# CAMMA-public/SelfPose3d

Measured on AMD Instinct MI355X. Metric: multi-view samples/sec (5-view Panoptic, 80x80x20 voxel), higher is better.
Workload: dtype f32

## Files before the change

### include/sp3d.h

```cpp
#ifndef SP3D_H
#define SP3D_H

#include <stdint.h>

#ifdef __cplusplus
extern "C" {
#endif

#define SP3D_ABI_VERSION 3
#define SP3D_MAX_VIEWS 16
#define SP3D_MAX_TOPK 32

#define SP3D_CAM_STRIDE 64
#define SP3D_CAM_R 0
#define SP3D_CAM_T 9
#define SP3D_CAM_F 12
#define SP3D_CAM_C 14
#define SP3D_CAM_K 16
#define SP3D_CAM_P 19
#define SP3D_CAM_A 21
#define SP3D_CAM_W0 27
#define SP3D_CAM_H0 28
#define SP3D_CAM_FLIP 29
#define SP3D_CAM_RXY 32
// ... 145 lines not shown
int sp3d_wino_input(const float *x, float *V, int B, int X, int Y, int Z, int C, void *stream);
int sp3d_wino_output(const float *M, float *y, const float *shift, const float *residual, int mode, int B, int X, int Y,
                     int Z, int O, void *stream);
int sp3d_wino_fused(const float *x, const float *U, float *y, const float *shift, const float *residual, int mode, int B,
                    int X, int Y, int Z, int C, int O, void *stream);

int sp3d_wino_fused_split(const float *x, const void *U3, float *y, const float *shift, const float *residual, int mode, int B,
                          int X, int Y, int Z, int C, int O, void *stream);

int sp3d_wino_fused_split64(const float *x, const void *U3, float *y, const float *shift, const float *residual, int mode,
                            int B, int X, int Y, int Z, int C, int O, void *stream);

int sp3d_conv3_split(const float *x, const void *W3, float *y, const float *shift, const float *residual, int mode, int B,
                     int X, int Y, int Z, int C, int O, void *stream);

int sp3d_upsample2x_scatter(const float *G, float *out, const float *shift, const float *skip, int64_t batch, int X, int Y,
                            int Z, int O, void *stream);

int sp3d_upsample2x_scatter_head(const float *G, float *head, const float *shift, const float *skip, const float *wout,
                                 const float *bout, int64_t batch, int X, int Y, int Z, int O, int J, void *stream);

#include "sp3d_upconv.h"

#define SP3D_GBN_F32 0
#define SP3D_GBN_F64 1
#define SP3D_GBN_REPLICAS 16
#define SP3D_GBN_PLAIN 0
#define SP3D_GBN_RELU 1
#define SP3D_GBN_ADD_RELU 2
int64_t sp3d_gbn_workspace_bytes(int G, int C);
// ... 14 lines not shown
```

### selfpose3d_amd/_lib.py

```python
from __future__ import annotations

import ctypes as C
import os
from typing import Optional, Sequence

import torch

_HERE = os.path.dirname(os.path.abspath(__file__))
_DEFAULT_LIB_PATH = os.path.join(_HERE, "libsp3d.so")
NOPK_LIB_PATH = os.path.join(_HERE, "libsp3d_nopk.so")
LIB_PATH = os.environ.get("SP3D_LIB_PATH") or _DEFAULT_LIB_PATH

LAYOUT_PLANAR = 0
LAYOUT_NHWC = 1
OUT_CHANNELS_LAST = 0x100
HM_BF16 = 0x200
OUT_BF16 = 0x400
HM_ONE_CHANNEL = 0x800
SCATTER_AUTO, SCATTER_PER_TAP, SCATTER_MERGE = 0, 2, 3
MAX_VIEWS = 16
MAX_TOPK = 32
ABI_VERSION = 3

_CTYPES = {"p": C.c_void_p, "i": C.c_int, "l": C.c_int64, "f": C.c_float, "d": C.c_double, "s": C.c_char_p}
# ... 53 lines not shown
}
TUNING_SIGNATURES = {
    "sp3d_unproject_fwd_variant": "i: p i ppppp iiiiiiii p iii p",
    "sp3d_unproject_fwd_plan": "i: iii p iiiiiiiii pppp",
    "sp3d_debug_set_timeline": "i: p",
    "sp3d_debug_stamp": "i: pp",
}
ONE_TRAIN_SIGNATURES = {
    "sp3d_unproject_one_fwd_train": "i: p ii ppppppp iiiiiiii p ii p",
    "sp3d_unproject_one_bwd": "i: ppppp l pp iiiiiiii p ii p",
    "sp3d_unproject_one_bwd_det": "i: ppppp l ppp iiiiiiii p ii p",
}
UPCONV_SIGNATURES = {
    "sp3d_upconv2x_fused": "i: ppppppp l iiiiii p",
}
EXPORTS = list(SIGNATURES)

_lib = None


class Sp3dError(RuntimeError):
    pass


def shared_gpu() -> bool:
    v = os.environ.get("SP3D_SHARED_GPU")
    if v is not None:
        return v.lower() in ("1", "true", "yes", "on")
    if any(os.environ.get(k) not in (None, "") for k in ("HIP_VISIBLE_DEVICES", "CUDA_VISIBLE_DEVICES", "ROCR_VISIBLE_DEVICES",
                                                          "GPU_DEVICE_ORDINAL")):
# ... 9 lines not shown
        pass
    return False


def load():
    global _lib, LIB_PATH
    if _lib is not None:
        return _lib
    if shared_gpu() and LIB_PATH == _DEFAULT_LIB_PATH:
        LIB_PATH = NOPK_LIB_PATH
    if not os.path.exists(LIB_PATH):
        raise Sp3dError(
            f"{LIB_PATH} not found - the HIP extension is not built. Run `python -m selfpose3d_amd.build` "
            "(hipcc, gfx950). There is no CPU fallback for the unprojection path.")
    lib = C.CDLL(LIB_PATH)
    for table, required in ((SIGNATURES, True), (ONE_TRAIN_SIGNATURES, True), (UPCONV_SIGNATURES, True),
                            (TUNING_SIGNATURES, False)):
        for name, sig in table.items():
            if required or hasattr(lib, name):
                ret, args = sig.split(":")
                fn = getattr(lib, name)
                fn.restype = _CTYPES[ret]
                fn.argtypes = [_CTYPES[a] for a in args.replace(" ", "")]
    if lib.sp3d_abi_version() != ABI_VERSION:
        raise Sp3dError(f"libsp3d.so ABI {lib.sp3d_abi_version()} != binding ABI {ABI_VERSION}; rebuild")
    _lib = lib
    return lib


def check(rc: int, what: str):
    if rc != 0:
# ... 603 lines not shown


def wino_weights_split(U: torch.Tensor, chunk: int = 8) -> torch.Tensor:
    P, Cc, O = (int(v) for v in U.shape)
    U = U.float()
    hi = U.bfloat16()
    r = U - hi.float()
    mid = r.bfloat16()
    lo = (r - mid.float()).bfloat16()
    pieces = torch.stack([mid, hi, lo], 0).reshape(3, P, Cc // chunk, chunk // 4, 4, O)
    return pieces.permute(1, 2, 3, 5, 0, 4).contiguous()


def conv_weights_split(w: torch.Tensor) -> torch.Tensor:
    O, Cc = int(w.shape[0]), int(w.shape[1])
    pc = wino_weights_split(w.float().permute(4, 3, 2, 1, 0).reshape(27, Cc, O).contiguous(), 8)
    mid, hi, lo = pc[..., 0, :], pc[..., 1, :], pc[..., 2, :]
    return torch.stack([hi, lo, hi, hi, mid, mid], -2).contiguous()


def conv3_split_(x: torch.Tensor, W3: torch.Tensor, shift: torch.Tensor, mode: int,
                 residual: Optional[torch.Tensor] = None) -> torch.Tensor:
    lib = load()
    _require_cuda(x, "x")
    B, Cc, X, Y, Z = (int(v) for v in x.shape)
    _require_cl3d_f32(x, "conv3_split_")
    O = int(W3.shape[3])
    dev = x.device
    y = _empty_cl3d(B, O, X, Y, Z, dev)
    if residual is not None:
        residual = _as_cl3d(residual)
    check(lib.sp3d_conv3_split(x.data_ptr(), W3.data_ptr(), y.data_ptr(), shift.data_ptr(), _opt(residual), int(mode),
                               B, X, Y, Z, Cc, O, _stream(dev)), "sp3d_conv3_split")
    return y


def wino_conv3d_(x: torch.Tensor, U: torch.Tensor, shift: torch.Tensor, mode: int,
                 residual: Optional[torch.Tensor] = None) -> torch.Tensor:
    lib = load()
    _require_cuda(x, "x")
    B, Cc, X, Y, Z = (int(v) for v in x.shape)
    _require_cl3d_f32(x, "wino_conv3d_")
    O = int(U.shape[2])
    T = B * ((X + 1) // 2) * ((Y + 1) // 2) * ((Z + 1) // 2)
    V = torch.empty((64, T, Cc), dtype=torch.float32, device=x.device)
    check(lib.sp3d_wino_input(x.data_ptr(), V.data_ptr(), B, X, Y, Z, Cc, _stream(x.device)), "sp3d_wino_input")
    M = torch.bmm(V, U)
    y = _empty_cl3d(B, O, X, Y, Z, x.device)
    if residual is not None:
        residual = _as_cl3d(residual)
    check(lib.sp3d_wino_output(M.data_ptr(), y.data_ptr(), shift.data_ptr(), _opt(residual), int(mode), B, X, Y, Z, O,
                               _stream(x.device)), "sp3d_wino_output")
    return y


def wino_fused_conv3d_(x: torch.Tensor, U: torch.Tensor, shift: torch.Tensor, mode: int,
                       residual: Optional[torch.Tensor] = None, U3: Optional[torch.Tensor] = None) -> torch.Tensor:
    lib = load()
    _require_cuda(x, "x")
    B, Cc, X, Y, Z = (int(v) for v in x.shape)
    _require_cl3d_f32(x, "wino_fused_conv3d_")
    O = int(U.shape[2])
    y = _empty_cl3d(B, O, X, Y, Z, x.device)
    if residual is not None:
        residual = _as_cl3d(residual)
    if U3 is None:
        name, weights = "sp3d_wino_fused", U
    else:
        name, weights = ("sp3d_wino_fused_split64" if O == 64 else "sp3d_wino_fused_split"), U3
    check(getattr(lib, name)(x.data_ptr(), weights.data_ptr(), y.data_ptr(), shift.data_ptr(), _opt(residual), int(mode),
                             B, X, Y, Z, Cc, O, _stream(x.device)), name)
    return y


def upconv_weights_split(w_gemm: torch.Tensor) -> torch.Tensor:
    Cc, O = int(w_gemm.shape[0]), int(w_gemm.shape[1]) // 8
    U = w_gemm.float().reshape(Cc, 8 * O // 32, 32).permute(1, 0, 2).contiguous()
    pc = wino_weights_split(U, 8)
# ... 92 lines not shown
```

### selfpose3d_amd/build.py

```python
from __future__ import annotations

import os
import subprocess
import sys

HERE = os.path.dirname(os.path.abspath(__file__))
CSRC = os.path.join(HERE, "csrc")
SOURCES = ["sp3d_unproject.hip", "sp3d_proposal.hip", "sp3d_epilogue.hip", "sp3d_upconv.hip", "sp3d_synth.hip", "sp3d_fftconv.hip", "sp3d_winograd.hip", "sp3d_fft.hip", "sp3d_gbn.hip"]
HEADERS = [os.path.join("..", "pk_src1.py"), "sp3d_device.h", "sp3d_proj_pk.h", "sp3d_split.h", "sp3d_tuning.h", "sp3d_twiddles.h", os.path.join("..", "..", "include", "sp3d.h"),
           os.path.join("..", "..", "include", "sp3d_one_train.h"), os.path.join("..", "..", "include", "sp3d_upconv.h")]
LIB = os.path.join(HERE, "libsp3d.so")
HIPCC = os.environ.get("HIPCC", "/opt/rocm/bin/hipcc")
FLAGS = ["--offload-arch=gfx950", "-O3", "-std=c++17", "-ffp-contract=off", "-munsafe-fp-atomics", "-fPIC", "-shared",
         "-Wall", "-Wno-unused-function"]
LINK = ["-L/opt/rocm/lib", "-lhipfft"]


def needs_build() -> bool:
    if not os.path.exists(LIB):
        return True
    t = os.path.getmtime(LIB)
    deps = [os.path.join(CSRC, s) for s in SOURCES + HEADERS] + [os.path.abspath(__file__)]
    return any(os.path.getmtime(d) > t for d in deps if os.path.exists(d))


# ... 102 lines not shown
```

### selfpose3d_amd/csrc/sp3d_winograd.hip

```cpp
#include <hip/hip_runtime.h>
#include <stdint.h>

#include "../../include/sp3d.h"
#include "sp3d_split.h"

namespace sp3d {

__device__ __forceinline__ void bt4(float &d0, float &d1, float &d2, float &d3)
{
    const float t0 = d0 - d2, t1 = d1 + d2, t2 = d2 - d1, t3 = d1 - d3;
    d0 = t0; d1 = t1; d2 = t2; d3 = t3;
}

__global__ __launch_bounds__(256) void wino_input_kernel(const float *__restrict__ x, float *__restrict__ V, int B, int X,
                                                        int Y, int Z, int C, int TX, int TY, int TZ)
{
    const int64_t T = (int64_t)B * TX * TY * TZ;
    const int64_t gid = (int64_t)blockIdx.x * 256 + threadIdx.x;
    if (gid >= T * C) return;
    const int c = (int)(gid % C);
    int64_t t = gid / C;
    const int tz = (int)(t % TZ); int64_t r = t / TZ;
    const int ty = (int)(r % TY); r /= TY;
    const int tx = (int)(r % TX);
// ... 526 lines not shown
                float val = acc[a][v] + sh;
                if (MODE == 2) val += rv[v];
                if (MODE >= 1) val = fmaxf(val, 0.0f);
                if (MODE == 3) val += rv[v];
                y[idx] = val;
            }
        }
    }
}

typedef float f32x4 __attribute__((ext_vector_type(4)));
constexpr int W16_RX = 10, W16_RY = 10, W16_RZ = 4, W16_VS = 16;
constexpr int W16_ROW = W16_RX * W16_VS + 4;
constexpr int W16_LDS = W16_RY * W16_RZ * W16_ROW;

__device__ __forceinline__ f32x4 mfma16_bf16(u32x4 a, u32x4 b, f32x4 c)
{
    return __builtin_amdgcn_mfma_f32_16x16x32_bf16(__builtin_bit_cast(bf16x8, a), __builtin_bit_cast(bf16x8, b), c, 0, 0, 0);
}

template <int C, int MODE, int NBW, int KS>
__global__ __launch_bounds__(64 * (4 / NBW) * KS) __attribute__((amdgpu_waves_per_eu(NBW <= 2 ? 2 : 1))) void wino_fused16_kernel(const float *__restrict__ x,
                                                                          const unsigned *__restrict__ U3,
                                                                          float *__restrict__ y, const float *__restrict__ shift,
                                                                          const float *__restrict__ res, int B, int X, int Y,
                                                                          int Z, int NBX, int NBY, int NBZ)
{
    constexpr int O = 64, NCH = C / 16, NOW = 4 / NBW, NTG = 64 * NOW;
    static_assert(NCH % KS == 0, "chunks must divide evenly over the channel groups");
    __shared__ __attribute__((aligned(16))) float lds[KS * W16_LDS];
    const int tid = threadIdx.x, lane = tid & 63, wave = tid >> 6;
    const int kg = wave / NOW, ow = wave % NOW, tg = tid - kg * NTG;
    float *region = lds + kg * W16_LDS;
    const int tl = lane & 15, q = lane >> 4;
    int bid = blockIdx.x;
    const int bz = bid % NBZ; bid /= NBZ;
    const int by = bid % NBY; bid /= NBY;
    const int bx = bid % NBX;
    const int b = bid / NBX;
    const int ttx = tl & 3, tty = tl >> 2;
    const int ox0 = bx * 8, oy0 = by * 8, oz0 = bz * 2;
// ... 146 lines not shown
                for (int bc = 0; bc < 4; ++bc) {
#if defined(SP3D_NO_PK) || defined(SP3D_W16_SCALAR_ACC)
                    for (int e = 0; e < 4; ++e) {
                        acc[bc][n][e] = fmaf(M0[n][e], cyz[bc], acc[bc][n][e]);
                        acc[4 + bc][n][e] = fmaf(M1[n][e], cyz[bc], acc[4 + bc][n][e]);
                    }
#else
                    const f32x4 cv = {cyz[bc], cyz[bc], cyz[bc], cyz[bc]};
                    acc[bc][n] = __builtin_elementwise_fma(M0[n], cv, acc[bc][n]);
                    acc[4 + bc][n] = __builtin_elementwise_fma(M1[n], cv, acc[4 + bc][n]);
#endif
                }
        }
    }

    if (KS > 1) {
        __syncthreads();
        f32x4 *red = reinterpret_cast<f32x4 *>(lds);
        if (kg > 0) {
#pragma unroll
            for (int a = 0; a < 8; ++a)
#pragma unroll
                for (int n = 0; n < NBW; ++n) red[(((kg - 1) * NOW + ow) * 8 * NBW + a * NBW + n) * 64 + lane] = acc[a][n];
        }
        __syncthreads();
        if (kg > 0) return;
#pragma unroll
        for (int g2 = 1; g2 < KS; ++g2)
#pragma unroll
            for (int a = 0; a < 8; ++a)
// ... 12 lines not shown
            for (int v = 0; v < 4; ++v) off[v] = ((2 * v * Y + 2 * q) * Z) * O;
            float rv[8][4];
            if (MODE >= 2) {
#pragma unroll
                for (int a = 0; a < 8; ++a)
#pragma unroll
                    for (int v = 0; v < 4; ++v)
                        rv[a][v] = res[obase + off[v] + (((a >> 2) * Y + ((a >> 1) & 1)) * Z + (a & 1)) * O];
            }
#pragma unroll
            for (int a = 0; a < 8; ++a)
#pragma unroll
                for (int v = 0; v < 4; ++v) {
                    float val = acc[a][n][v] + sh;
                    if (MODE == 2) val += rv[a][v];
                    if (MODE >= 1) val = fmaxf(val, 0.0f);
                    if (MODE == 3) val += rv[a][v];
                    y[obase + off[v] + (((a >> 2) * Y + ((a >> 1) & 1)) * Z + (a & 1)) * O] = val;
                }
        }
        return;
    }
#pragma unroll
    for (int n = 0; n < NBW; ++n) {
        const int o = (ow * NBW + n) * 16 + tl;
        const float sh = shift[o];
        float rv[8][4];
        if (MODE >= 2) {
#pragma unroll
            for (int a = 0; a < 8; ++a)
#pragma unroll
// ... 4 lines not shown
                    const int zo = min(oz0 + (a & 1), Z - 1);
                    rv[a][v] = res[((((int64_t)b * X + xo) * Y + yo) * Z + zo) * O + o];
                }
        }
#pragma unroll
        for (int a = 0; a < 8; ++a) {
#pragma unroll
            for (int v = 0; v < 4; ++v) {
                const int tile = 4 * q + v;
                const int rx = tile & 3, ry = tile >> 2;
                const int xo = ox0 + 2 * rx + (a >> 2), yo = oy0 + 2 * ry + ((a >> 1) & 1), zo = oz0 + (a & 1);
                if (xo < X && yo < Y && zo < Z) {
                    const int64_t idx = ((((int64_t)b * X + xo) * Y + yo) * Z + zo) * O + o;
                    float val = acc[a][n][v] + sh;
                    if (MODE == 2) val += rv[a][v];
                    if (MODE >= 1) val = fmaxf(val, 0.0f);
                    if (MODE == 3) val += rv[a][v];
                    y[idx] = val;
                }
            }
        }
    }
}


constexpr int CD_BX = 16, CD_BY = 8, CD_BZ = 4;
constexpr int CD_RX = CD_BX + 2, CD_RY = CD_BY + 2, CD_RZ = CD_BZ + 2, CD_VOX = 8, CD_ROW = CD_RX * CD_VOX, CD_ZP = CD_RY * CD_ROW + 4;
constexpr int CD_PLANE = CD_RZ * CD_ZP;
constexpr int CD_BUF = 2 * CD_PLANE;
constexpr int CD_NV4 = CD_RX * CD_RY * CD_RZ * 2;
constexpr int CD_PROD = 4;
// ... 3 lines not shown
#define SP3D_WG_ABLATE 0
#endif
struct CdRec { u32x4 hl, hh, mm; };


#ifdef SP3D_CD_TIMELINE
__device__ unsigned long long *g_cd_tl = nullptr;
#define CD_STAMP(slot) do { __builtin_amdgcn_sched_barrier(0); if (g_cd_tl && blockIdx.x == 0 && lane == 0 && item < 64) { g_cd_tl[(wave * 64 + item) * 4 + (slot)] = __builtin_readcyclecounter(); \
     \
    if (wave == 0 && (slot) == 0 && item == 0) { g_cd_tl[(7 * 64 + 62) * 4 + 0] = wall_clock64(); g_cd_tl[(7 * 64 + 62) * 4 + 1] = __builtin_readcyclecounter(); } \
    if (wave == 0 && (slot) == 3) { g_cd_tl[(7 * 64 + 63) * 4 + 0] = wall_clock64(); g_cd_tl[(7 * 64 + 63) * 4 + 1] = __builtin_readcyclecounter(); } } __builtin_amdgcn_sched_barrier(0); } while (0)
#else
#define CD_STAMP(slot) do { (void)item; } while (0)
#endif

template <int C, int MODE>
__global__ __launch_bounds__(64 * (4 + CD_PROD)) __attribute__((amdgpu_waves_per_eu(2, 2)))
void conv3_split_kernel(const float *__restrict__ x, const unsigned *__restrict__ W3, float *__restrict__ y,
                        const float *__restrict__ shift, const float *__restrict__ res, int B, int X, int Y, int Z, int NBX,
                        int NBY, int NBZ, int nblocks)
{
    constexpr int O = 32, NCH = C / 8;
    extern __shared__ __attribute__((aligned(16))) unsigned cd_lds[];
    const int tid = threadIdx.x, lane = tid & 63, wave = tid >> 6, t = lane & 31, h = lane >> 5;
    const int my_blocks = ((int)blockIdx.x < nblocks) ? (nblocks - 1 - (int)blockIdx.x) / (int)gridDim.x + 1 : 0;
    const int n_items = my_blocks * NCH;
    auto decode = [&](int item, int &b, int &ox0, int &oy0, int &oz0) {
        int bid = (int)blockIdx.x + (item / NCH) * (int)gridDim.x;
        const int bz = bid % NBZ; bid /= NBZ;
        const int by = bid % NBY; bid /= NBY;
        const int bx = bid % NBX;
        b = bid / NBX;
        ox0 = bx * CD_BX; oy0 = by * CD_BY; oz0 = bz * CD_BZ;
    };

    if (wave >= 4) {
        const int pt = tid - 256;
// ... 85 lines not shown
#pragma unroll
                for (int v = 0; v < 16; ++v) acc[m][v] = 0.0f;
        }
        auto load_a = [&](int st, Opnd &a) {
            const int dz = st / 3, dy = st % 3;
#pragma unroll
            for (int j = 0; j < 6; ++j) {
                const unsigned *p = ab + dz * CD_ZP + dy * CD_ROW + j * CD_VOX;
                a.lh[j] = *reinterpret_cast<const u32x4 *>(p);
                a.hm[j] = *reinterpret_cast<const u32x4 *>(p + 4);
            }
        };
        Opnd a0, a1;
        load_a(0, a0);
        const int q0 = item * 9;
        CD_STAMP(0);
#pragma unroll
        for (int st = 0; st < 9; ++st) {
            __builtin_amdgcn_sched_barrier(0);
            w1 = load_w(min(q0 + st + 1, n_items * 9 - 1));
            if (st + 1 < 9) load_a(st + 1, a1);
#pragma unroll
            for (int dx = 0; dx < 3; ++dx) {
#pragma unroll
                for (int i = 0; i < 4; ++i) acc[i] = mfma_bf16(a0.lh[i + dx], w0.d[dx].hl, acc[i]);
#pragma unroll
                for (int i = 0; i < 4; ++i) acc[i] = mfma_bf16(a0.hm[i + dx], w0.d[dx].hh, acc[i]);
#pragma unroll
                for (int i = 0; i < 4; ++i) acc[i] = mfma_bf16(a0.hm[i + dx], w0.d[dx].mm, acc[i]);
            }
#pragma unroll
            for (int r = 0; r < 12; ++r) {
                __builtin_amdgcn_sched_group_barrier(0x008, 1, 0);
                __builtin_amdgcn_sched_group_barrier(0x100, 1, 0);
            }
#pragma unroll
            for (int r = 0; r < 9; ++r) {
                __builtin_amdgcn_sched_group_barrier(0x008, 1, 0);
                __builtin_amdgcn_sched_group_barrier(0x020, 1, 0);
            }
            __builtin_amdgcn_sched_group_barrier(0x008, 15, 0);
            __builtin_amdgcn_sched_barrier(0);
            a0 = a1;
            w0 = w1;
        }
        CD_STAMP(1);
        if (cc == NCH - 1) {
            int b, ox0, oy0, oz0;
            decode(item, b, ox0, oy0, oz0);
            if (ox0 + CD_BX <= X && oy0 + CD_BY <= Y && oz0 + CD_BZ <= Z) {
                const float sh = shift[t];
                const int64_t obase = ((((int64_t)b * X + ox0 + 4 * wave) * Y + oy0 + 4 * h) * Z + oz0) * O + t;
#pragma unroll
                for (int i = 0; i < 4; ++i)
#pragma unroll
                    for (int v = 0; v < 16; ++v) {
                        const int64_t idx = obase + (((int64_t)i * Y + (v & 3)) * Z + (v >> 2)) * O;
                        float val = acc[i][v] + sh;
                        if (MODE == 2) val += res[idx];
                        if (MODE >= 1) val = fmaxf(val, 0.0f);
                        if (MODE == 3) val += res[idx];
#if SP3D_W16_ABLATE & 16
                        if (val == 123.456f)
#endif
                        y[idx] = val;
                    }
            } else {
            float *scr = reinterpret_cast<float *>(cd_lds + 2 * CD_BUFS) + wave * 1024;
            const int g = lane & 7;
            const float4 sh4 = *reinterpret_cast<const float4 *>(shift + 4 * g);
#pragma unroll
            for (int mb = 0; mb < 4; ++mb) {
#pragma unroll
                for (int v = 0; v < 16; ++v) scr[(8 * (v >> 2) + (v & 3) + 4 * h) * 32 + t] = acc[mb][v];
                __builtin_amdgcn_fence(__ATOMIC_RELEASE, "wavefront");
                __builtin_amdgcn_wave_barrier();
#pragma unroll
                for (int r = 0; r < 4; ++r) {
                    const int m = (lane >> 3) + 8 * r;
                    float4 a = *reinterpret_cast<const float4 *>(scr + m * 32 + 4 * g);
                    const int xo = ox0 + 4 * wave + mb, yo = oy0 + (m & 7), zo = oz0 + (m >> 3);
                    if (xo < X && yo < Y && zo < Z) {
                        const int64_t vox = (((int64_t)b * X + xo) * Y + yo) * Z + zo;
                        a.x += sh4.x; a.y += sh4.y; a.z += sh4.z; a.w += sh4.w;
                        float4 rr = make_float4(0.0f, 0.0f, 0.0f, 0.0f);
                        if (MODE >= 2) rr = *reinterpret_cast<const float4 *>(res + vox * O + 4 * g);
                        if (MODE == 2) { a.x += rr.x; a.y += rr.y; a.z += rr.z; a.w += rr.w; }
                        if (MODE >= 1) { a.x = fmaxf(a.x, 0.0f); a.y = fmaxf(a.y, 0.0f); a.z = fmaxf(a.z, 0.0f); a.w = fmaxf(a.w, 0.0f); }
                        if (MODE == 3) { a.x += rr.x; a.y += rr.y; a.z += rr.z; a.w += rr.w; }
#if SP3D_W16_ABLATE & 16
                        if (a.x == 123.456f)
#endif
                        *reinterpret_cast<float4 *>(y + vox * O + 4 * g) = a;
                    }
                }
                __builtin_amdgcn_fence(__ATOMIC_RELEASE, "wavefront");
                __builtin_amdgcn_wave_barrier();
            }
            }
        }
        CD_STAMP(2);
        __syncthreads();
        CD_STAMP(3);
// ... 59 lines not shown

extern "C" int sp3d_wino_fused_split64(const float *x, const void *U3, float *y, const float *shift, const float *residual,
                                       int mode, int B, int X, int Y, int Z, int C, int O, void *stream)
{
    using namespace sp3d;
    if (B <= 0 || X <= 0 || Y <= 0 || Z <= 0 || mode < 0 || mode > 3) return SP3D_EINVAL;
    if (!x || !U3 || !y || !shift || (mode >= 2 && !residual)) return SP3D_ENULL;
    if (O != 64 || (C != 32 && C != 64) || (reinterpret_cast<uintptr_t>(U3) & 7)) return SP3D_EUNSUPPORTED;
    const int NBX = (X + 7) / 8, NBY = (Y + 7) / 8, NBZ = (Z + 1) / 2;
    const int64_t blocks = (int64_t)B * NBX * NBY * NBZ;
    if (blocks > 0x7fffffff) return SP3D_ERANGE;
    constexpr int nbw = 2, ks = 2;
    hipStream_t s = (hipStream_t)stream;
    const unsigned *u3 = reinterpret_cast<const unsigned *>(U3);
    const dim3 grid((unsigned)blocks), block(64 * (4 / nbw) * ks);
#define SP3D_WF(C_, M_) hipLaunchKernelGGL((wino_fused16_kernel<C_, M_, 2, 2>), grid, block, 0, s, x, u3, y, shift, residual, B, X, Y, Z, NBX, NBY, NBZ)
#define SP3D_WFM(C_) switch (mode) { case 0: SP3D_WF(C_, 0); break; case 1: SP3D_WF(C_, 1); break; case 2: SP3D_WF(C_, 2); break; default: SP3D_WF(C_, 3); }
    if (C == 32) { SP3D_WFM(32) } else { SP3D_WFM(64) }
#undef SP3D_WFM
#undef SP3D_WF
    const hipError_t e = hipGetLastError();
    return e == hipSuccess ? SP3D_OK : (int)e;
}

extern "C" int sp3d_conv3_split(const float *x, const void *W3, float *y, const float *shift, const float *residual, int mode,
                                int B, int X, int Y, int Z, int C, int O, void *stream)
{
    using namespace sp3d;
    if (B <= 0 || X <= 0 || Y <= 0 || Z <= 0 || mode < 0 || mode > 3) return SP3D_EINVAL;
    if (!x || !W3 || !y || !shift || (mode >= 2 && !residual)) return SP3D_ENULL;
    if (O != 32 || (C != 16 && C != 32) || (reinterpret_cast<uintptr_t>(W3) & 15)) return SP3D_EUNSUPPORTED;
    if (reinterpret_cast<uintptr_t>(y) & 15) return SP3D_EUNSUPPORTED;
    if ((int64_t)X * Y * Z * C * 2 > 0x7fffffff) return SP3D_ERANGE;
    const int NBX = (X + CD_BX - 1) / CD_BX, NBY = (Y + CD_BY - 1) / CD_BY, NBZ = (Z + CD_BZ - 1) / CD_BZ;
    const int64_t blocks = (int64_t)B * NBX * NBY * NBZ;
    if (blocks > 0x7fffffff) return SP3D_ERANGE;
    static int cu_count[64] = {0};
    int dev = 0, cus = 256;
    if (hipGetDevice(&dev) == hipSuccess && dev >= 0 && dev < 64) {
        if (cu_count[dev] == 0) {
            int n = 0;
            cu_count[dev] = (hipDeviceGetAttribute(&n, hipDeviceAttributeMultiprocessorCount, dev) == hipSuccess && n > 0) ? n : 256;
        }
        cus = cu_count[dev];
    }
    const int rounds = (int)((blocks + cus - 1) / cus);
    const int nwg = (int)((blocks + rounds - 1) / rounds);
    const dim3 grid((unsigned)nwg), block(64 * (4 + CD_PROD));
    const size_t lds = (size_t)2 * CD_BUFS * sizeof(unsigned) + 4 * 1024 * sizeof(float);
    hipStream_t s = (hipStream_t)stream;
    const unsigned *w3 = reinterpret_cast<const unsigned *>(W3);
    int cd_dev = 0;
    { const hipError_t ed = hipGetDevice(&cd_dev); if (ed != hipSuccess) return (int)ed; }
    if (cd_dev < 0 || cd_dev >= 64) cd_dev = 63;
#define SP3D_CD(C_, M_) { static bool attr_dev[64] = {}; bool &attr = attr_dev[cd_dev]; if (!attr || cd_dev == 63) { hipError_t ea = hipFuncSetAttribute(reinterpret_cast<const void *>(conv3_split_kernel<C_, M_>), hipFuncAttributeMaxDynamicSharedMemorySize, (int)lds); if (ea != hipSuccess) return (int)ea; attr = true; } \
    hipLaunchKernelGGL((conv3_split_kernel<C_, M_>), grid, block, lds, s, x, w3, y, shift, residual, B, X, Y, Z, NBX, NBY, NBZ, (int)blocks); }
#define SP3D_CDI(C_) switch (mode) { case 0: SP3D_CD(C_, 0); break; case 1: SP3D_CD(C_, 1); break; case 2: SP3D_CD(C_, 2); break; default: SP3D_CD(C_, 3); }
    if (C == 16) { SP3D_CDI(16) } else { SP3D_CDI(32) }
#undef SP3D_CDI
#undef SP3D_CD
    const hipError_t e = hipGetLastError();
    return e == hipSuccess ? SP3D_OK : (int)e;
}

extern "C" int sp3d_debug_conv3_timeline(void *dev_buffer)
{
#ifdef SP3D_CD_TIMELINE
    unsigned long long *p = (unsigned long long *)dev_buffer;
    return (int)hipMemcpyToSymbol(HIP_SYMBOL(sp3d::g_cd_tl), &p, sizeof(p));
#else
    (void)dev_buffer;
    return SP3D_EUNSUPPORTED;
#endif
}
```

### selfpose3d_amd/v2v_net.py

```python
from __future__ import annotations

from typing import NamedTuple, Optional

import torch
import torch.nn as nn
import torch.nn.functional as F


def _bn(c):
    from .grouped_bn import GroupedBatchNorm3d
    return GroupedBatchNorm3d(c)


def _grouped(bn, training: bool) -> bool:
    return training and getattr(bn, "groups", None) is not None


def fft_len(n: int) -> int:
    m = n + (n & 1)
    while True:
        r, odd = m, 0
        for q in (2, 3, 5, 7, 11, 13):
            if q > 2 and r % q == 0:
                odd += 1
# ... 181 lines not shown
        self.device, self.is_cuda, self.dtype = spec.device, spec.is_cuda, torch.float32


class _Conv(NamedTuple):
    w: torch.Tensor
    shift: torch.Tensor
    u: Optional[torch.Tensor] = None
    split: Optional[torch.Tensor] = None
    direct: Optional[torch.Tensor] = None


class _Res(NamedTuple):
    c1: _Conv
    c2: _Conv
    skip: Optional[torch.Tensor]


class _Up(NamedTuple):
    wT: torch.Tensor
    shift: torch.Tensor
    wg: torch.Tensor
    split: Optional[torch.Tensor] = None


class _FoldedV2V:

    def __init__(self, net: "V2VNet"):
        self.net = net
        self.key = None
        self.layers = {}
# ... 34 lines not shown
        u = _lib.wino_weights(w)
        split = _lib.wino_weights_split(u, 16 if cout == 64 else 8) if "wino_fused_conv3d_" in routes else None
        direct = _lib.conv_weights_split(w) if "conv3_split_" in routes else None
        return _Conv(w, shift, u, split, direct)

    def _build(self):
        from . import _lib
        n, layers = self.net, {}
        layers["front"] = _Conv(*self._fold(n.front_layers[0].block[0], n.front_layers[0].block[1]))
        ed = n.encoder_decoder
        for name in ("front_res", "encoder_res1", "encoder_res2", "mid_res", "decoder_res2", "decoder_res1", "skip_res1",
                     "skip_res2"):
            blk = n.front_layers[1] if name == "front_res" else getattr(ed, name)
            w1, s1 = self._fold(blk.res_branch[0], blk.res_branch[1])
            w2, s2 = self._fold(blk.res_branch[3], blk.res_branch[4])
            ws = None
            if len(blk.skip_con) > 0:
                ws, ss = self._fold(blk.skip_con[0], blk.skip_con[1])
                s2 = (s2 + ss).contiguous()
            layers[name] = _Res(self._conv3_record(w1, s1), self._conv3_record(w2, s2), ws)
        for name in ("decoder_upsample2", "decoder_upsample1"):
            blk = getattr(ed, name).block
            wT, sT = self._fold(blk[0], blk[1], transposed=True)
            wg = wT.permute(0, 2, 3, 4, 1).reshape(wT.shape[0], 8 * wT.shape[1]).contiguous()
            fused = wg.is_cuda and (int(wT.shape[0]), int(wT.shape[1])) in ((128, 64), (64, 32))
            layers[name] = _Up(wT, sT, wg, _lib.upconv_weights_split(wg) if fused else None)
        self.layers, self.spectra, self.xpad = layers, {}, {}

    def _conv3(self, x, c: "_Conv", mode, residual=None):
        from . import _lib
        n, route = self.net, "library"
        split = getattr(n, "wino_split", True)
        if c.u is not None and is_cl(x):
            route = conv3_route(int(c.w.shape[1]), int(c.w.shape[0]), (x.shape[0],) + tuple(x.shape[2:]), n.winograd, split,
                                getattr(n, "direct_conv", True))
        if route == "conv3_split_":
            return _lib.conv3_split_(x, c.direct, c.shift, mode, residual)
        if route == "wino_fused_conv3d_":
            return _lib.wino_fused_conv3d_(x, c.u, c.shift, mode, residual, c.split if split else None)
        if route == "wino_conv3d_":
            return _lib.wino_conv3d_(x, c.u, c.shift, mode, residual)
        return _lib.channel_shift_act_(F.conv3d(x, c.w, None, 1, 1), c.shift, mode, residual)

    def _res(self, x, name):
        r = self.layers[name]
        h = self._conv3(x, r.c1, 1)
        return self._conv3(h, r.c2, 2, x if r.skip is None else self._conv1(x, r.skip))

    _tuned_shapes: "set[tuple]" = set()
    _tune_gemms = None

    @staticmethod
    def _tunable():
        import os
        on = _FoldedV2V._tune_gemms
        if on is None:
            on = os.environ.get("SP3D_TUNE_GEMM", "0") not in ("0", "")
        return getattr(torch.cuda, "tunable", None) if on else None

    def _run_tuned(self, x):
        tun = self._tunable()
        if tun is None or not x.is_cuda:
# ... 287 lines not shown
```

Baseline: 2802.

## Fold 1x1x1 skip-projection conv into the second residual 3x3x3 conv kernel

For residual blocks with a projection skip (16->32 and 32->64 channels), the 1x1x1 skip convolution is folded into the epilogue of the second 3x3x3 conv, in both the direct split-bf16 kernel and the 64-channel Winograd kernel. The skip's split-precision weights are precomputed, and extra bf16 MFMAs accumulate x_skip*W_skip into the same accumulators before shift+ReLU. This removes a separate conv1 launch plus the write and read of the residual tensor. The cost is more registers and loads inside the conv kernels, which may lower occupancy, and ReLU now keeps NaNs on the skip path.

```diff
diff --git a/include/sp3d.h b/include/sp3d.h
--- a/include/sp3d.h
+++ b/include/sp3d.h
@@ -183,6 +183,8 @@
 int sp3d_conv3_split(const float *x, const void *W3, float *y, const float *shift, const float *residual, int mode, int B,
                      int X, int Y, int Z, int C, int O, void *stream);
 
+#include "sp3d_skip_fold.h"
+
 int sp3d_upsample2x_scatter(const float *G, float *out, const float *shift, const float *skip, int64_t batch, int X, int Y,
                             int Z, int O, void *stream);
 
diff --git a/include/sp3d_skip_fold.h b/include/sp3d_skip_fold.h
--- /dev/null
+++ b/include/sp3d_skip_fold.h
@@ -0,0 +1,10 @@
+#ifndef SP3D_SKIP_FOLD_H
+#define SP3D_SKIP_FOLD_H
+
+int sp3d_conv3_split_skip(const float *x, const void *W3, float *y, const float *shift, const float *xs, const void *WS,
+                          int B, int X, int Y, int Z, int C, int O, int CS, void *stream);
+
+int sp3d_wino_fused_split64_skip(const float *x, const void *U3, float *y, const float *shift, const float *xs, const void *WS,
+                                 int B, int X, int Y, int Z, int C, int O, int CS, void *stream);
+
+#endif
diff --git a/selfpose3d_amd/_lib.py b/selfpose3d_amd/_lib.py
--- a/selfpose3d_amd/_lib.py
+++ b/selfpose3d_amd/_lib.py
@@ -91,6 +91,10 @@
 UPCONV_SIGNATURES = {
     "sp3d_upconv2x_fused": "i: ppppppp l iiiiii p",
 }
+SKIP_FOLD_SIGNATURES = {
+    "sp3d_conv3_split_skip": "i: pppppp iiiiiii p",
+    "sp3d_wino_fused_split64_skip": "i: pppppp iiiiiii p",
+}
 EXPORTS = list(SIGNATURES)
 
 _lib = None
@@ -130,7 +134,7 @@
             f"{LIB_PATH} not found - the HIP extension is not built. Run `python -m selfpose3d_amd.build` "
             "(hipcc, gfx950). There is no CPU fallback for the unprojection path.")
     lib = C.CDLL(LIB_PATH)
-    for table, required in ((SIGNATURES, True), (ONE_TRAIN_SIGNATURES, True), (UPCONV_SIGNATURES, True),
+    for table, required in ((SIGNATURES, True), (ONE_TRAIN_SIGNATURES, True), (UPCONV_SIGNATURES, True), (SKIP_FOLD_SIGNATURES, True),
                             (TUNING_SIGNATURES, False)):
         for name, sig in table.items():
             if required or hasattr(lib, name):
@@ -764,13 +768,28 @@
 
 def conv_weights_split(w: torch.Tensor) -> torch.Tensor:
     O, Cc = int(w.shape[0]), int(w.shape[1])
-    pc = wino_weights_split(w.float().permute(4, 3, 2, 1, 0).reshape(27, Cc, O).contiguous(), 8)
+    taps = int(w.shape[2]) * int(w.shape[3]) * int(w.shape[4])
+    pc = wino_weights_split(w.float().permute(4, 3, 2, 1, 0).reshape(taps, Cc, O).contiguous(), 8)
     mid, hi, lo = pc[..., 0, :], pc[..., 1, :], pc[..., 2, :]
     return torch.stack([hi, lo, hi, hi, mid, mid], -2).contiguous()
 
 
+def skip_fold_enabled() -> bool:
+    return os.environ.get("SP3D_FOLD_SKIP", "1") not in ("0", "")
+
+
+def _require_skip(xs: torch.Tensor, skip_w: torch.Tensor, x: torch.Tensor, CS: int, numel: int, who: str):
+    _require_cl3d_f32(xs, who)
+    if xs.device != x.device or tuple(xs.shape) != (x.shape[0], CS) + tuple(x.shape[2:]):
+        raise Sp3dError(f"{who}: xs must be ({x.shape[0]}, {CS}, ...) on the grid and device of x, got {tuple(xs.shape)} on {xs.device}")
+    if skip_w.device != x.device or skip_w.dtype != torch.bfloat16 or not skip_w.is_contiguous() or skip_w.numel() != numel:
+        raise Sp3dError(f"{who}: skip_w must be the split records of the ({x.shape[1]}, {CS}, 1, 1, 1) weight on {x.device}; got "
+                        f"{tuple(skip_w.shape)}, {skip_w.dtype}, {skip_w.device}, contiguous={skip_w.is_contiguous()}")
+
+
 def conv3_split_(x: torch.Tensor, W3: torch.Tensor, shift: torch.Tensor, mode: int,
-                 residual: Optional[torch.Tensor] = None) -> torch.Tensor:
+                 residual: Optional[torch.Tensor] = None, *, xs: Optional[torch.Tensor] = None,
+                 skip_w: Optional[torch.Tensor] = None) -> torch.Tensor:
     lib = load()
     _require_cuda(x, "x")
     B, Cc, X, Y, Z = (int(v) for v in x.shape)
@@ -778,6 +797,14 @@
     O = int(W3.shape[3])
     dev = x.device
     y = _empty_cl3d(B, O, X, Y, Z, dev)
+    if xs is not None or skip_w is not None:
+        if xs is None or skip_w is None or int(mode) != 1 or residual is not None:
+            raise Sp3dError("conv3_split_: the folded skip takes xs AND skip_w, mode 1 and no residual")
+        CS = 16
+        _require_skip(xs, skip_w, x, CS, CS * O * 6, "conv3_split_")
+        check(lib.sp3d_conv3_split_skip(x.data_ptr(), W3.data_ptr(), y.data_ptr(), shift.data_ptr(), xs.data_ptr(),
+                                        skip_w.data_ptr(), B, X, Y, Z, Cc, O, CS, _stream(dev)), "sp3d_conv3_split_skip")
+        return y
     if residual is not None:
         residual = _as_cl3d(residual)
     check(lib.sp3d_conv3_split(x.data_ptr(), W3.data_ptr(), y.data_ptr(), shift.data_ptr(), _opt(residual), int(mode),
@@ -805,13 +832,23 @@
 
 
 def wino_fused_conv3d_(x: torch.Tensor, U: torch.Tensor, shift: torch.Tensor, mode: int,
-                       residual: Optional[torch.Tensor] = None, U3: Optional[torch.Tensor] = None) -> torch.Tensor:
+                       residual: Optional[torch.Tensor] = None, U3: Optional[torch.Tensor] = None, *,
+                       xs: Optional[torch.Tensor] = None, skip_w: Optional[torch.Tensor] = None) -> torch.Tensor:
     lib = load()
     _require_cuda(x, "x")
     B, Cc, X, Y, Z = (int(v) for v in x.shape)
     _require_cl3d_f32(x, "wino_fused_conv3d_")
     O = int(U.shape[2])
     y = _empty_cl3d(B, O, X, Y, Z, x.device)
+    if xs is not None or skip_w is not None:
+        if xs is None or skip_w is None or U3 is None or int(mode) != 1 or residual is not None:
+            raise Sp3dError("wino_fused_conv3d_: the folded skip takes U3, xs AND skip_w, mode 1 and no residual")
+        CS = 32
+        _require_skip(xs, skip_w, x, CS, CS * O * 3, "wino_fused_conv3d_")
+        check(lib.sp3d_wino_fused_split64_skip(x.data_ptr(), U3.data_ptr(), y.data_ptr(), shift.data_ptr(), xs.data_ptr(),
+                                               skip_w.data_ptr(), B, X, Y, Z, Cc, O, CS, _stream(x.device)),
+              "sp3d_wino_fused_split64_skip")
+        return y
     if residual is not None:
         residual = _as_cl3d(residual)
     if U3 is None:
diff --git a/selfpose3d_amd/build.py b/selfpose3d_amd/build.py
--- a/selfpose3d_amd/build.py
+++ b/selfpose3d_amd/build.py
@@ -8,7 +8,8 @@
 CSRC = os.path.join(HERE, "csrc")
 SOURCES = ["sp3d_unproject.hip", "sp3d_proposal.hip", "sp3d_epilogue.hip", "sp3d_upconv.hip", "sp3d_synth.hip", "sp3d_fftconv.hip", "sp3d_winograd.hip", "sp3d_fft.hip", "sp3d_gbn.hip"]
 HEADERS = [os.path.join("..", "pk_src1.py"), "sp3d_device.h", "sp3d_proj_pk.h", "sp3d_split.h", "sp3d_tuning.h", "sp3d_twiddles.h", os.path.join("..", "..", "include", "sp3d.h"),
-           os.path.join("..", "..", "include", "sp3d_one_train.h"), os.path.join("..", "..", "include", "sp3d_upconv.h")]
+           os.path.join("..", "..", "include", "sp3d_one_train.h"), os.path.join("..", "..", "include", "sp3d_upconv.h"),
+           os.path.join("..", "..", "include", "sp3d_skip_fold.h")]
 LIB = os.path.join(HERE, "libsp3d.so")
 HIPCC = os.environ.get("HIPCC", "/opt/rocm/bin/hipcc")
 FLAGS = ["--offload-arch=gfx950", "-O3", "-std=c++17", "-ffp-contract=off", "-munsafe-fp-atomics", "-fPIC", "-shared",
diff --git a/selfpose3d_amd/csrc/sp3d_winograd.hip b/selfpose3d_amd/csrc/sp3d_winograd.hip
--- a/selfpose3d_amd/csrc/sp3d_winograd.hip
+++ b/selfpose3d_amd/csrc/sp3d_winograd.hip
@@ -564,17 +564,21 @@
 constexpr int W16_ROW = W16_RX * W16_VS + 4;
 constexpr int W16_LDS = W16_RY * W16_RZ * W16_ROW;
 
+__device__ __forceinline__ float relu_keep_nan(float v) { return v < 0.0f ? 0.0f : v; }
+
 __device__ __forceinline__ f32x4 mfma16_bf16(u32x4 a, u32x4 b, f32x4 c)
 {
     return __builtin_amdgcn_mfma_f32_16x16x32_bf16(__builtin_bit_cast(bf16x8, a), __builtin_bit_cast(bf16x8, b), c, 0, 0, 0);
 }
 
-template <int C, int MODE, int NBW, int KS>
+template <int C, int MODE, int NBW, int KS, bool SKIP = false>
 __global__ __launch_bounds__(64 * (4 / NBW) * KS) __attribute__((amdgpu_waves_per_eu(NBW <= 2 ? 2 : 1))) void wino_fused16_kernel(const float *__restrict__ x,
                                                                           const unsigned *__restrict__ U3,
                                                                           float *__restrict__ y, const float *__restrict__ shift,
                                                                           const float *__restrict__ res, int B, int X, int Y,
-                                                                          int Z, int NBX, int NBY, int NBZ)
+                                                                          int Z, int NBX, int NBY, int NBZ,
+                                                                          const float *__restrict__ xs = nullptr,
+                                                                          const unsigned *__restrict__ WS = nullptr)
 {
     constexpr int O = 64, NCH = C / 16, NOW = 4 / NBW, NTG = 64 * NOW;
     static_assert(NCH % KS == 0, "chunks must divide evenly over the channel groups");
@@ -751,6 +755,42 @@
         }
     }
 
+    if (SKIP) {
+        constexpr int CS = 32;
+        static_assert(!SKIP || KS * 16 == CS, "one skip chunk per channel group");
+        int ln = lane;
+        asm volatile("" : "+v"(ln));
+        const int stl = ln & 15, sq = ln >> 4;
+        const float *xsb = xs + (int64_t)b * X * Y * Z * CS + 16 * kg + 4 * sq;
+        float4 sx[8];
+#pragma unroll
+        for (int a = 0; a < 8; ++a) {
+            const int xo = min(ox0 + 2 * (stl & 3) + (a >> 2), X - 1), yo = min(oy0 + 2 * (stl >> 2) + ((a >> 1) & 1), Y - 1);
+            const int zo = min(oz0 + (a & 1), Z - 1);
+            sx[a] = *reinterpret_cast<const float4 *>(xsb + ((xo * Y + yo) * Z + zo) * CS);
+        }
+        WfB sw[NBW];
+#pragma unroll
+        for (int n = 0; n < NBW; ++n) {
+            const unsigned *r = WS + ((kg * 4 + sq) * O + (ow * NBW + n) * 16 + stl) * 6;
+            sw[n].mh = *reinterpret_cast<const u32x4_a8 *>(r);
+            sw[n].l = *reinterpret_cast<const u32x2_a8 *>(r + 4);
+        }
+#pragma unroll
+        for (int a = 0; a < 8; ++a) {
+            const u32x6 p = split3_pieces(sx[a]);
+            const u32x4 Qlh = split3_q0(p), Qhh = {p[2], p[3], p[2], p[3]}, Qmm = {p[4], p[5], p[4], p[5]};
+#pragma unroll
+            for (int n = 0; n < NBW; ++n) {
+                const u32x4 Bmh = sw[n].mh;
+                const u32x4 Bhl = {sw[n].mh.z, sw[n].mh.w, sw[n].l.x, sw[n].l.y};
+                acc[a][n] = mfma16_bf16(Qhh, Bmh, acc[a][n]);
+                acc[a][n] = mfma16_bf16(Qmm, Bmh, acc[a][n]);
+                acc[a][n] = mfma16_bf16(Qlh, Bhl, acc[a][n]);
+            }
+        }
+    }
+
     if (KS > 1) {
         __syncthreads();
         f32x4 *red = reinterpret_cast<f32x4 *>(lds);
@@ -793,7 +833,7 @@
                 for (int v = 0; v < 4; ++v) {
                     float val = acc[a][n][v] + sh;
                     if (MODE == 2) val += rv[a][v];
-                    if (MODE >= 1) val = fmaxf(val, 0.0f);
+                    if (MODE >= 1) val = SKIP ? relu_keep_nan(val) : fmaxf(val, 0.0f);
                     if (MODE == 3) val += rv[a][v];
                     y[obase + off[v] + (((a >> 2) * Y + ((a >> 1) & 1)) * Z + (a & 1)) * O] = val;
                 }
@@ -828,7 +868,7 @@
                     const int64_t idx = ((((int64_t)b * X + xo) * Y + yo) * Z + zo) * O + o;
                     float val = acc[a][n][v] + sh;
                     if (MODE == 2) val += rv[a][v];
-                    if (MODE >= 1) val = fmaxf(val, 0.0f);
+                    if (MODE >= 1) val = SKIP ? relu_keep_nan(val) : fmaxf(val, 0.0f);
                     if (MODE == 3) val += rv[a][v];
                     y[idx] = val;
                 }
@@ -862,13 +902,14 @@
 #define CD_STAMP(slot) do { (void)item; } while (0)
 #endif
 
-template <int C, int MODE>
+template <int C, int MODE, bool SKIP = false>
 __global__ __launch_bounds__(64 * (4 + CD_PROD)) __attribute__((amdgpu_waves_per_eu(2, 2)))
 void conv3_split_kernel(const float *__restrict__ x, const unsigned *__restrict__ W3, float *__restrict__ y,
                         const float *__restrict__ shift, const float *__restrict__ res, int B, int X, int Y, int Z, int NBX,
-                        int NBY, int NBZ, int nblocks)
-{
-    constexpr int O = 32, NCH = C / 8;
+                        int NBY, int NBZ, int nblocks, const float *__restrict__ xs = nullptr,
+                        const unsigned *__restrict__ WS = nullptr)
+{
+    constexpr int O = 32, NCH = C / 8, CS = 16;
     extern __shared__ __attribute__((aligned(16))) unsigned cd_lds[];
     const int tid = threadIdx.x, lane = tid & 63, wave = tid >> 6, t = lane & 31, h = lane >> 5;
     const int my_blocks = ((int)blockIdx.x < nblocks) ? (nblocks - 1 - (int)blockIdx.x) / (int)gridDim.x + 1 : 0;
@@ -984,9 +1025,23 @@
         Opnd a0, a1;
         load_a(0, a0);
         const int q0 = item * 9;
+        float s0[4];
+        unsigned so[4];
         CD_STAMP(0);
 #pragma unroll
         for (int st = 0; st < 9; ++st) {
+            if (SKIP && st == 8 && cc == NCH - 1) {
+                int b, ox0, oy0, oz0;
+                decode(item, b, ox0, oy0, oz0);
+                const float *xb = xs + (int64_t)b * X * Y * Z * CS;
+                const int ys = min(oy0 + (t & 7), Y - 1), zs = min(oz0 + (t >> 3), Z - 1);
+#pragma unroll
+                for (int i = 0; i < 4; ++i) {
+                    const int xv = min(ox0 + 4 * wave + i, X - 1);
+                    so[i] = (unsigned)(((xv * Y + ys) * Z + zs) * CS + 4 * h);
+                    s0[i] = xb[so[i]];
+                }
+            }
             __builtin_amdgcn_sched_barrier(0);
             w1 = load_w(min(q0 + st + 1, n_items * 9 - 1));
             if (st + 1 < 9) load_a(st + 1, a1);
@@ -1015,6 +1070,41 @@
             w0 = w1;
         }
         CD_STAMP(1);
+        if (SKIP && cc == NCH - 1) {
+            float4 sv[2][4];
+            {
+                int b, ox0, oy0, oz0;
+                decode(item, b, ox0, oy0, oz0);
+                const float *xb = xs + (int64_t)b * X * Y * Z * CS;
+#pragma unroll
+                for (int i = 0; i < 4; ++i) {
+                    const float *p = xb + so[i];
+                    sv[0][i] = make_float4(s0[i], p[1], p[2], p[3]);
+                    sv[1][i] = *reinterpret_cast<const float4 *>(p + 8);
+                }
+            }
+            CdRec ws[2];
+#pragma unroll
+            for (int c2 = 0; c2 < 2; ++c2) {
+                const unsigned *r = WS + (unsigned)(((c2 * 2 + h) * O + t) * 12);
+                ws[c2].hl = *reinterpret_cast<const u32x4 *>(r);
+                ws[c2].hh = *reinterpret_cast<const u32x4 *>(r + 4);
+                ws[c2].mm = *reinterpret_cast<const u32x4 *>(r + 8);
+            }
+#pragma unroll
+            for (int c2 = 0; c2 < 2; ++c2) {
+                __builtin_amdgcn_sched_barrier(0);
+                u32x4 lh[4], hm[4];
+#pragma unroll
+                for (int i = 0; i < 4; ++i) split3(sv[c2][i], lh[i], hm[i]);
+#pragma unroll
+                for (int i = 0; i < 4; ++i) acc[i] = mfma_bf16(lh[i], ws[c2].hl, acc[i]);
+#pragma unroll
+                for (int i = 0; i < 4; ++i) acc[i] = mfma_bf16(hm[i], ws[c2].hh, acc[i]);
+#pragma unroll
+                for (int i = 0; i < 4; ++i) acc[i] = mfma_bf16(hm[i], ws[c2].mm, acc[i]);
+            }
+        }
         if (cc == NCH - 1) {
             int b, ox0, oy0, oz0;
             decode(item, b, ox0, oy0, oz0);
@@ -1028,7 +1118,7 @@
                         const int64_t idx = obase + (((int64_t)i * Y + (v & 3)) * Z + (v >> 2)) * O;
                         float val = acc[i][v] + sh;
                         if (MODE == 2) val += res[idx];
-                        if (MODE >= 1) val = fmaxf(val, 0.0f);
+                        if (MODE >= 1) val = SKIP ? relu_keep_nan(val) : fmaxf(val, 0.0f);
                         if (MODE == 3) val += res[idx];
 #if SP3D_W16_ABLATE & 16
                         if (val == 123.456f)
@@ -1056,7 +1146,8 @@
                         float4 rr = make_float4(0.0f, 0.0f, 0.0f, 0.0f);
                         if (MODE >= 2) rr = *reinterpret_cast<const float4 *>(res + vox * O + 4 * g);
                         if (MODE == 2) { a.x += rr.x; a.y += rr.y; a.z += rr.z; a.w += rr.w; }
-                        if (MODE >= 1) { a.x = fmaxf(a.x, 0.0f); a.y = fmaxf(a.y, 0.0f); a.z = fmaxf(a.z, 0.0f); a.w = fmaxf(a.w, 0.0f); }
+                        if (MODE >= 1 && SKIP) { a.x = relu_keep_nan(a.x); a.y = relu_keep_nan(a.y); a.z = relu_keep_nan(a.z); a.w = relu_keep_nan(a.w); }
+                        if (MODE >= 1 && !SKIP) { a.x = fmaxf(a.x, 0.0f); a.y = fmaxf(a.y, 0.0f); a.z = fmaxf(a.z, 0.0f); a.w = fmaxf(a.w, 0.0f); }
                         if (MODE == 3) { a.x += rr.x; a.y += rr.y; a.z += rr.z; a.w += rr.w; }
 #if SP3D_W16_ABLATE & 16
                         if (a.x == 123.456f)
@@ -1146,7 +1237,7 @@
     hipStream_t s = (hipStream_t)stream;
     const unsigned *u3 = reinterpret_cast<const unsigned *>(U3);
     const dim3 grid((unsigned)blocks), block(64 * (4 / nbw) * ks);
-#define SP3D_WF(C_, M_) hipLaunchKernelGGL((wino_fused16_kernel<C_, M_, 2, 2>), grid, block, 0, s, x, u3, y, shift, residual, B, X, Y, Z, NBX, NBY, NBZ)
+#define SP3D_WF(C_, M_) hipLaunchKernelGGL((wino_fused16_kernel<C_, M_, 2, 2>), grid, block, 0, s, x, u3, y, shift, residual, B, X, Y, Z, NBX, NBY, NBZ, (const float *)nullptr, (const unsigned *)nullptr)
 #define SP3D_WFM(C_) switch (mode) { case 0: SP3D_WF(C_, 0); break; case 1: SP3D_WF(C_, 1); break; case 2: SP3D_WF(C_, 2); break; default: SP3D_WF(C_, 3); }
     if (C == 32) { SP3D_WFM(32) } else { SP3D_WFM(64) }
 #undef SP3D_WFM
@@ -1155,15 +1246,10 @@
     return e == hipSuccess ? SP3D_OK : (int)e;
 }
 
-extern "C" int sp3d_conv3_split(const float *x, const void *W3, float *y, const float *shift, const float *residual, int mode,
-                                int B, int X, int Y, int Z, int C, int O, void *stream)
+static int conv3_split_launch(const float *x, const void *W3, float *y, const float *shift, const float *residual, int mode,
+                              const float *xs, const void *WS, int B, int X, int Y, int Z, int C, void *stream)
 {
     using namespace sp3d;
-    if (B <= 0 || X <= 0 || Y <= 0 || Z <= 0 || mode < 0 || mode > 3) return SP3D_EINVAL;
-    if (!x || !W3 || !y || !shift || (mode >= 2 && !residual)) return SP3D_ENULL;
-    if (O != 32 || (C != 16 && C != 32) || (reinterpret_cast<uintptr_t>(W3) & 15)) return SP3D_EUNSUPPORTED;
-    if (reinterpret_cast<uintptr_t>(y) & 15) return SP3D_EUNSUPPORTED;
-    if ((int64_t)X * Y * Z * C * 2 > 0x7fffffff) return SP3D_ERANGE;
     const int NBX = (X + CD_BX - 1) / CD_BX, NBY = (Y + CD_BY - 1) / CD_BY, NBZ = (Z + CD_BZ - 1) / CD_BZ;
     const int64_t blocks = (int64_t)B * NBX * NBY * NBZ;
     if (blocks > 0x7fffffff) return SP3D_ERANGE;
@@ -1181,18 +1267,61 @@
     const dim3 grid((unsigned)nwg), block(64 * (4 + CD_PROD));
     const size_t lds = (size_t)2 * CD_BUFS * sizeof(unsigned) + 4 * 1024 * sizeof(float);
     hipStream_t s = (hipStream_t)stream;
-    const unsigned *w3 = reinterpret_cast<const unsigned *>(W3);
+    const unsigned *w3 = reinterpret_cast<const unsigned *>(W3), *wsk = reinterpret_cast<const unsigned *>(WS);
     int cd_dev = 0;
     { const hipError_t ed = hipGetDevice(&cd_dev); if (ed != hipSuccess) return (int)ed; }
     if (cd_dev < 0 || cd_dev >= 64) cd_dev = 63;
-#define SP3D_CD(C_, M_) { static bool attr_dev[64] = {}; bool &attr = attr_dev[cd_dev]; if (!attr || cd_dev == 63) { hipError_t ea = hipFuncSetAttribute(reinterpret_cast<const void *>(conv3_split_kernel<C_, M_>), hipFuncAttributeMaxDynamicSharedMemorySize, (int)lds); if (ea != hipSuccess) return (int)ea; attr = true; } \
-    hipLaunchKernelGGL((conv3_split_kernel<C_, M_>), grid, block, lds, s, x, w3, y, shift, residual, B, X, Y, Z, NBX, NBY, NBZ, (int)blocks); }
-#define SP3D_CDI(C_) switch (mode) { case 0: SP3D_CD(C_, 0); break; case 1: SP3D_CD(C_, 1); break; case 2: SP3D_CD(C_, 2); break; default: SP3D_CD(C_, 3); }
-    if (C == 16) { SP3D_CDI(16) } else { SP3D_CDI(32) }
+#define SP3D_CD(C_, M_, S_) { static bool attr_dev[64] = {}; bool &attr = attr_dev[cd_dev]; if (!attr || cd_dev == 63) { hipError_t ea = hipFuncSetAttribute(reinterpret_cast<const void *>(conv3_split_kernel<C_, M_, S_>), hipFuncAttributeMaxDynamicSharedMemorySize, (int)lds); if (ea != hipSuccess) return (int)ea; attr = true; } \
+    hipLaunchKernelGGL((conv3_split_kernel<C_, M_, S_>), grid, block, lds, s, x, w3, y, shift, residual, B, X, Y, Z, NBX, NBY, NBZ, (int)blocks, xs, wsk); }
+#define SP3D_CDI(C_) switch (mode) { case 0: SP3D_CD(C_, 0, false); break; case 1: SP3D_CD(C_, 1, false); break; case 2: SP3D_CD(C_, 2, false); break; default: SP3D_CD(C_, 3, false); }
+    if (xs) { SP3D_CD(32, 1, true) } else if (C == 16) { SP3D_CDI(16) } else { SP3D_CDI(32) }
 #undef SP3D_CDI
 #undef SP3D_CD
     const hipError_t e = hipGetLastError();
     return e == hipSuccess ? SP3D_OK : (int)e;
+}
+
+extern "C" int sp3d_wino_fused_split64_skip(const float *x, const void *U3, float *y, const float *shift, const float *xs,
+                                            const void *WS, int B, int X, int Y, int Z, int C, int O, int CS, void *stream)
+{
+    using namespace sp3d;
+    if (B <= 0 || X <= 0 || Y <= 0 || Z <= 0) return SP3D_EINVAL;
+    if (!x || !U3 || !y || !shift || !xs || !WS) return SP3D_ENULL;
+    if (O != 64 || C != 64 || CS != 32 || (reinterpret_cast<uintptr_t>(U3) & 7)) return SP3D_EUNSUPPORTED;
+    if ((reinterpret_cast<uintptr_t>(WS) & 7) || (reinterpret_cast<uintptr_t>(xs) & 15)) return SP3D_EUNSUPPORTED;
+    if ((int64_t)X * Y * Z * CS > 0x7fffffff) return SP3D_ERANGE;
+    const int NBX = (X + 7) / 8, NBY = (Y + 7) / 8, NBZ = (Z + 1) / 2;
+    const int64_t blocks = (int64_t)B * NBX * NBY * NBZ;
+    if (blocks > 0x7fffffff) return SP3D_ERANGE;
+    hipStream_t s = (hipStream_t)stream;
+    const dim3 grid((unsigned)blocks), block(64 * 2 * 2);
+    hipLaunchKernelGGL((wino_fused16_kernel<64, 1, 2, 2, true>), grid, block, 0, s, x, reinterpret_cast<const unsigned *>(U3), y, shift,
+                       (const float *)nullptr, B, X, Y, Z, NBX, NBY, NBZ, xs, reinterpret_cast<const unsigned *>(WS));
+    const hipError_t e = hipGetLastError();
+    return e == hipSuccess ? SP3D_OK : (int)e;
+}
+
+extern "C" int sp3d_conv3_split(const float *x, const void *W3, float *y, const float *shift, const float *residual, int mode,
+                                int B, int X, int Y, int Z, int C, int O, void *stream)
+{
+    if (B <= 0 || X <= 0 || Y <= 0 || Z <= 0 || mode < 0 || mode > 3) return SP3D_EINVAL;
+    if (!x || !W3 || !y || !shift || (mode >= 2 && !residual)) return SP3D_ENULL;
+    if (O != 32 || (C != 16 && C != 32) || (reinterpret_cast<uintptr_t>(W3) & 15)) return SP3D_EUNSUPPORTED;
+    if (reinterpret_cast<uintptr_t>(y) & 15) return SP3D_EUNSUPPORTED;
+    if ((int64_t)X * Y * Z * C * 2 > 0x7fffffff) return SP3D_ERANGE;
+    return conv3_split_launch(x, W3, y, shift, residual, mode, nullptr, nullptr, B, X, Y, Z, C, stream);
+}
+
+extern "C" int sp3d_conv3_split_skip(const float *x, const void *W3, float *y, const float *shift, const float *xs,
+                                     const void *WS, int B, int X, int Y, int Z, int C, int O, int CS, void *stream)
+{
+    if (B <= 0 || X <= 0 || Y <= 0 || Z <= 0) return SP3D_EINVAL;
+    if (!x || !W3 || !y || !shift || !xs || !WS) return SP3D_ENULL;
+    if (O != 32 || C != 32 || CS != 16) return SP3D_EUNSUPPORTED;
+    if ((reinterpret_cast<uintptr_t>(W3) | reinterpret_cast<uintptr_t>(WS) | reinterpret_cast<uintptr_t>(xs) |
+         reinterpret_cast<uintptr_t>(y)) & 15) return SP3D_EUNSUPPORTED;
+    if ((int64_t)X * Y * Z * C * 2 > 0x7fffffff) return SP3D_ERANGE;
+    return conv3_split_launch(x, W3, y, shift, nullptr, 1, xs, WS, B, X, Y, Z, C, stream);
 }
 
 extern "C" int sp3d_debug_conv3_timeline(void *dev_buffer)
diff --git a/selfpose3d_amd/v2v_net.py b/selfpose3d_amd/v2v_net.py
--- a/selfpose3d_amd/v2v_net.py
+++ b/selfpose3d_amd/v2v_net.py
@@ -219,6 +219,8 @@
     c1: _Conv
     c2: _Conv
     skip: Optional[torch.Tensor]
+    skip_direct: Optional[torch.Tensor] = None
+    skip_split: Optional[torch.Tensor] = None
 
 
 class _Up(NamedTuple):
@@ -283,11 +285,16 @@
             blk = n.front_layers[1] if name == "front_res" else getattr(ed, name)
             w1, s1 = self._fold(blk.res_branch[0], blk.res_branch[1])
             w2, s2 = self._fold(blk.res_branch[3], blk.res_branch[4])
-            ws = None
+            ws = sd = sp = None
             if len(blk.skip_con) > 0:
                 ws, ss = self._fold(blk.skip_con[0], blk.skip_con[1])
                 s2 = (s2 + ss).contiguous()
-            layers[name] = _Res(self._conv3_record(w1, s1), self._conv3_record(w2, s2), ws)
+                co, ci = int(ws.shape[0]), int(ws.shape[1])
+                if ws.is_cuda and (co, ci) == (32, 16):
+                    sd = _lib.conv_weights_split(ws)
+                if ws.is_cuda and (co, ci) == (64, 32):
+                    sp = _lib.wino_weights_split(ws.reshape(co, ci).t().reshape(1, ci, co).contiguous(), 16)
+            layers[name] = _Res(self._conv3_record(w1, s1), self._conv3_record(w2, s2), ws, sd, sp)
         for name in ("decoder_upsample2", "decoder_upsample1"):
             blk = getattr(ed, name).block
             wT, sT = self._fold(blk[0], blk[1], transposed=True)
@@ -296,25 +303,46 @@
             layers[name] = _Up(wT, sT, wg, _lib.upconv_weights_split(wg) if fused else None)
         self.layers, self.spectra, self.xpad = layers, {}, {}
 
-    def _conv3(self, x, c: "_Conv", mode, residual=None):
-        from . import _lib
-        n, route = self.net, "library"
-        split = getattr(n, "wino_split", True)
-        if c.u is not None and is_cl(x):
-            route = conv3_route(int(c.w.shape[1]), int(c.w.shape[0]), (x.shape[0],) + tuple(x.shape[2:]), n.winograd, split,
-                                getattr(n, "direct_conv", True))
+    def _route(self, x, c: "_Conv") -> str:
+        n = self.net
+        if c.u is None or not is_cl(x):
+            return "library"
+        return conv3_route(int(c.w.shape[1]), int(c.w.shape[0]), (x.shape[0],) + tuple(x.shape[2:]), n.winograd,
+                           getattr(n, "wino_split", True), getattr(n, "direct_conv", True))
+
+    def _conv3(self, x, c: "_Conv", mode, residual=None, xs=None, skip_w=None):
+        from . import _lib
+        route = self._route(x, c)
+        split = getattr(self.net, "wino_split", True)
         if route == "conv3_split_":
-            return _lib.conv3_split_(x, c.direct, c.shift, mode, residual)
+            return _lib.conv3_split_(x, c.direct, c.shift, mode, residual, xs=xs, skip_w=skip_w)
         if route == "wino_fused_conv3d_":
-            return _lib.wino_fused_conv3d_(x, c.u, c.shift, mode, residual, c.split if split else None)
+            return _lib.wino_fused_conv3d_(x, c.u, c.shift, mode, residual, c.split if split else None, xs=xs, skip_w=skip_w)
+        assert xs is None and skip_w is None, route
         if route == "wino_conv3d_":
             return _lib.wino_conv3d_(x, c.u, c.shift, mode, residual)
         return _lib.channel_shift_act_(F.conv3d(x, c.w, None, 1, 1), c.shift, mode, residual)
 
+    def _folded_skip(self, x, h, r: "_Res"):
+        from . import _lib
+        if r.skip is None or not _lib.skip_fold_enabled() or not (is_cl(x) and x.is_cuda and x.dtype == torch.float32):
+            return None
+        route, widths = self._route(h, r.c2), (int(r.c2.w.shape[1]), int(r.c2.w.shape[0]), int(x.shape[1]))
+        if route == "conv3_split_" and widths == (32, 32, 16):
+            return r.skip_direct
+        if route == "wino_fused_conv3d_" and getattr(self.net, "wino_split", True) and widths == (64, 64, 32):
+            return r.skip_split
+        return None
+
     def _res(self, x, name):
         r = self.layers[name]
         h = self._conv3(x, r.c1, 1)
-        return self._conv3(h, r.c2, 2, x if r.skip is None else self._conv1(x, r.skip))
+        if r.skip is None:
+            return self._conv3(h, r.c2, 2, x)
+        rec = self._folded_skip(x, h, r)
+        if rec is not None:
+            return self._conv3(h, r.c2, 1, xs=x, skip_w=rec)
+        return self._conv3(h, r.c2, 2, self._conv1(x, r.skip))
 
     _tuned_shapes: "set[tuple]" = set()
     _tune_gemms = None
```

After: 2834 (median of 6 runs). 1.1% higher.
